# ignaschuemer7/soft-actor-critic

Hardware: AMD Instinct MI355X
Metric: SAC gradient steps/sec + replay-sample GB/s, BipedalWalker batch=256 (higher is better)
Workload: dtype fp32; 1 GPU; c2: BipedalWalker-v3 obs=24 act=4 2x[256, 256] MLPs, buffer=1000000, batch=256, auto-alpha, device sampler, fp32 arithmetic; global_batch=256, parallelism=replicas1, graph_chunk=64

## Files before the change

### soft-actor-critic_amd/csrc/sac_engine.hip

```cpp
#include "../../include/sac_engine.h"
#include "../../include/sac_engine_testing.h"

#include <algorithm>
#include <math.h>
#include <stdio.h>
#include <stdlib.h>
#include <string.h>
#include <string>
#include <vector>

#define SAC_VERSION "sac-mi355x 0.1.0"

#include "sac_phases.h"
#include "sac_split.h"
#include "sac_wide.h"
#include "sac_pairs.h"
#include "sac_envs.h"
#include "sac_plan.h"

template <typename T>
__global__ void pack_weights(const float* __restrict__ W, int K, int N, int Kp, int Np, T* __restrict__ Wc,
                             T* __restrict__ WTc) {
  for (int i = blockIdx.x * blockDim.x + threadIdx.x; i < Np * Kp; i += gridDim.x * blockDim.x) {
    const int n = i / Kp, k = i % Kp;
// ... 184 lines not shown

__host__ __device__ inline void eps_pair(uint64_t seed, uint64_t step, int b, int which, int p, int B, int A,
                                         float* out) {
  float n0, n1;
  philox_normal2(seed, step, (uint32_t)b, (uint32_t)which, (uint32_t)p, n0, n1);
  float* o = out + ((size_t)which * B + b) * A;
  o[2 * p] = n0;
  if (2 * p + 1 < A) o[2 * p + 1] = n1;
}
__global__ void eps_draw_kernel(uint64_t seed, uint64_t step, int B, int A, float* __restrict__ out) {
  const int NP = (A + 1) / 2;
  const int64_t n = 2LL * B * NP;
  for (int64_t i = blockIdx.x * (int64_t)blockDim.x + threadIdx.x; i < n; i += (int64_t)gridDim.x * blockDim.x) {
    const int p = (int)(i % NP);
    const int64_t rw = i / NP;
    eps_pair(seed, step, (int)(rw % B), (int)(rw / B), p, B, A, out);
  }
}

__global__ void replay_sample_kernel(const int64_t* __restrict__ state, int B, FeistelKeys fk, int32_t* __restrict__ out) {
  const int64_t size = state[0];
  const Feistel f = feistel_from_keys(fk, size);
  for (int b = blockIdx.x * blockDim.x + threadIdx.x; b < B; b += gridDim.x * blockDim.x)
    out[b] = (int32_t)feistel_sample(f, b, size);
}

static thread_local std::string g_err;
static int fail(int code, const std::string& msg) {
  g_err = msg;
  return code;
}
#define HIPCHK(x)                                                                                  \
  do {                                                                                             \
    hipError_t _e = (x);                                                                           \
    if (_e != hipSuccess) return fail(SAC_E_HIP, std::string(#x ": ") + hipGetErrorString(_e));    \
  } while (0)

static int validate(const sac_engine_config* c) {
  if (!c) return fail(SAC_E_INVALID, "null config");
  if (c->obs_dim < 1 || c->act_dim < 1 || c->act_dim > 32) return fail(SAC_E_INVALID, "obs_dim >= 1, 1 <= act_dim <= 32");
  if (c->batch < 1 || c->batch > (1 << 20)) return fail(SAC_E_INVALID, "batch out of range");
  if (c->q_layers < 2 || c->q_layers > SAC_DEV_LAYERS || c->pi_layers < 2 || c->pi_layers > SAC_DEV_LAYERS)
    return fail(SAC_E_INVALID, "networks need 1..5 hidden layers");
  if (c->q_dims[0] != c->obs_dim + c->act_dim || c->q_dims[c->q_layers] != 1)
    return fail(SAC_E_INVALID, "q_dims must run obs+act -> ... -> 1");
  if (c->pi_dims[0] != c->obs_dim || c->pi_dims[c->pi_layers] != 2 * c->act_dim)
    return fail(SAC_E_INVALID, "pi_dims must run obs -> ... -> 2*act");
  for (int i = 0; i <= c->q_layers; ++i)
    if (c->q_dims[i] < 1) return fail(SAC_E_INVALID, "bad q dim");
  for (int i = 0; i <= c->pi_layers; ++i)
    if (c->pi_dims[i] < 1) return fail(SAC_E_INVALID, "bad pi dim");
  const int acts[4] = {c->q_hidden_act, c->q_out_act, c->pi_hidden_act, c->pi_out_act};
  for (int a : acts)
    if (a < 0 || a > 6) return fail(SAC_E_INVALID, "bad activation code");
  if (c->precision != SAC_PREC_FP32 && c->precision != SAC_PREC_BF16) return fail(SAC_E_INVALID, "bad precision");
  if (c->layout < SAC_LAYOUT_AUTO || c->layout > SAC_LAYOUT_PAIRS || c->stage_path < -1 || c->stage_path > 1 ||
      c->stage_batch < -1 || c->stage_batch > 0 || c->upd_parts < 0 || c->upd_parts > 4 ||
      (c->upd_threads != 0 && c->upd_threads != 512 && c->upd_threads != 1024))
    return fail(SAC_E_INVALID, "bad layout override (layout 0..3, stage_path -1..1, stage_batch -1..0, "
                               "upd_parts 0..4, upd_threads 0 / 512 / 1024)");
  return SAC_OK;
}

template <typename T>
static void set_lds_attrs(size_t bytes) {
  (void)bytes;
  const int b = 160 * 1024;
  (void)hipFuncSetAttribute((const void*)sac_target_critic<T, false>, hipFuncAttributeMaxDynamicSharedMemorySize, b);
  (void)hipFuncSetAttribute((const void*)sac_target_critic<T, true>, hipFuncAttributeMaxDynamicSharedMemorySize, b);
  (void)hipFuncSetAttribute((const void*)sac_actor<T, false>, hipFuncAttributeMaxDynamicSharedMemorySize, b);
  (void)hipFuncSetAttribute((const void*)sac_actor<T, true>, hipFuncAttributeMaxDynamicSharedMemorySize, b);
  (void)hipFuncSetAttribute((const void*)sac_policy_act_kernel<T>, hipFuncAttributeMaxDynamicSharedMemorySize, b);
  (void)hipFuncSetAttribute((const void*)sac_rollout_step_kernel<T, false>, hipFuncAttributeMaxDynamicSharedMemorySize, b);
  (void)hipFuncSetAttribute((const void*)sac_rollout_step_kernel<T, true>, hipFuncAttributeMaxDynamicSharedMemorySize, b);
  (void)hipFuncSetAttribute((const void*)sac_rollout_step_dev_kernel<T, false>, hipFuncAttributeMaxDynamicSharedMemorySize,
                            b);
  (void)hipFuncSetAttribute((const void*)sac_rollout_step_dev_kernel<T, true>, hipFuncAttributeMaxDynamicSharedMemorySize,
                            b);
  (void)hipFuncSetAttribute((const void*)sac_q_values_kernel<T>, hipFuncAttributeMaxDynamicSharedMemorySize, b);
  (void)hipFuncSetAttribute((const void*)sac_target_critic_split<T>, hipFuncAttributeMaxDynamicSharedMemorySize, b);
  (void)hipFuncSetAttribute((const void*)sac_target_critic_pairs<T>, hipFuncAttributeMaxDynamicSharedMemorySize, b);
  (void)hipFuncSetAttribute((const void*)sac_actor_pairs<T>, hipFuncAttributeMaxDynamicSharedMemorySize, b);
  (void)hipFuncSetAttribute((const void*)sac_actor_split<T>, hipFuncAttributeMaxDynamicSharedMemorySize, b);
  (void)hipFuncSetAttribute((const void*)sac_critic_update<T>, hipFuncAttributeMaxDynamicSharedMemorySize, b);
  (void)hipFuncSetAttribute((const void*)sac_critic_update<T, 512>, hipFuncAttributeMaxDynamicSharedMemorySize, b);
  (void)hipFuncSetAttribute((const void*)sac_actor_update<T>, hipFuncAttributeMaxDynamicSharedMemorySize, b);
  (void)hipFuncSetAttribute((const void*)sac_wide_stage<T, WA_PLAIN, false>, hipFuncAttributeMaxDynamicSharedMemorySize, b);
  (void)hipFuncSetAttribute((const void*)sac_wide_stage<T, WA_ACT, false>, hipFuncAttributeMaxDynamicSharedMemorySize, b);
  (void)hipFuncSetAttribute((const void*)sac_wide_stage<T, WA_OUTBWD, false>, hipFuncAttributeMaxDynamicSharedMemorySize, b);
  (void)hipFuncSetAttribute((const void*)sac_wide_stage<T, WA_PLAIN, true>, hipFuncAttributeMaxDynamicSharedMemorySize, b);
  (void)hipFuncSetAttribute((const void*)sac_wide_stage<T, WA_ACT, true>, hipFuncAttributeMaxDynamicSharedMemorySize, b);
  (void)hipFuncSetAttribute((const void*)sac_wide_stage<T, WA_OUTBWD, true>, hipFuncAttributeMaxDynamicSharedMemorySize, b);
  (void)hipFuncSetAttribute((const void*)sac_wide_gather<T>, hipFuncAttributeMaxDynamicSharedMemorySize, b);
  (void)hipFuncSetAttribute((const void*)sac_wide_head<T>, hipFuncAttributeMaxDynamicSharedMemorySize, b);
}

__global__ void sac_noop_kernel() {}
__global__ void sac_spin_kernel(long long ticks) {
  const long long t0 = __builtin_amdgcn_s_memrealtime();
  while (__builtin_amdgcn_s_memrealtime() - t0 < ticks) __builtin_amdgcn_s_sleep(8);
}

#define BY_PRECISION(e, fn, ...) \
  ((e)->cfg.precision == SAC_PREC_BF16 ? fn<bf16>(__VA_ARGS__) : fn<float>(__VA_ARGS__))

template <typename T>
static void launch_kind(sac_engine* e, int kind, const sac_replay* rb, const int32_t* idx, const float* eps,
                        hipStream_t s) {
  const PhaseLaunch& L = e->launch[kind];
  switch (kind) {
    case L_A:
      switch (e->path) {
        case PATH_SPLIT: sac_target_critic_split<T><<<L.grid, L.threads, L.lds, s>>>(e->d, *rb, idx, eps); break;
        case PATH_ROLES: sac_target_critic<T, true><<<L.grid, L.threads, L.lds, s>>>(e->d, *rb, idx, eps); break;
        case PATH_PAIRS: sac_target_critic_pairs<T><<<L.grid, L.threads, L.lds, s>>>(e->d, *rb, idx, eps); break;
        case PATH_ROWS: sac_target_critic<T, false><<<L.grid, L.threads, L.lds, s>>>(e->d, *rb, idx, eps); break;
        case PATH_WIDE: break;
      }
      break;
    case L_B:
      if (L.threads == 512)
        sac_critic_update<T, 512><<<L.grid, 512, L.lds, s>>>(e->d, e->tilesB);
      else
        sac_critic_update<T><<<L.grid, L.threads, L.lds, s>>>(e->d, e->tilesB);
      break;
    case L_C:
      switch (e->path) {
        case PATH_SPLIT: sac_actor_split<T><<<L.grid, L.threads, L.lds, s>>>(e->d, *rb); break;
        case PATH_ROLES: sac_actor<T, true><<<L.grid, L.threads, L.lds, s>>>(e->d, *rb); break;
        case PATH_PAIRS: sac_actor_pairs<T><<<L.grid, L.threads, L.lds, s>>>(e->d, *rb); break;
        case PATH_ROWS: sac_actor<T, false><<<L.grid, L.threads, L.lds, s>>>(e->d, *rb); break;
        case PATH_WIDE: break;
      }
      break;
    case L_D:
      sac_actor_update<T><<<L.grid, L.threads, L.lds, s>>>(e->d, e->tilesD, e->nD);
      break;
  }
}

template <typename T>
static void launch_wide_stage(sac_engine* e, const sac_engine::WStage& st, const sac_replay* rb, const int32_t* idx,
                              const float* eps, hipStream_t s, bool stage_next, const int32_t* next_idx) {
  const size_t glds = (size_t)((WGR * (e->cfg.obs_dim + e->cfg.act_dim) + 1) & ~1) * 4 + WGR * 8;
  switch (st.kind) {
    case 0:
      sac_wide_gather<T><<<st.grid, WG_T, glds, s>>>(e->d, e->wdd, *rb, idx);
      break;
    case 1: {
      const int ng = st.last && stage_next ? (e->cfg.batch + WGR - 1) / WGR : 0;
      const int flags = st.last | (&st == &e->wst[1] ? 2 : 0) | (ng ? 4 : 0) | (int)((&st - e->wst.data()) << 8);
      const bool relu = e->cfg.q_hidden_act == ACT_RELU && e->cfg.pi_hidden_act == ACT_RELU;
      const int am = e->hostW[st.j0].amode;
      auto k = relu ? (am == WA_PLAIN ? sac_wide_stage<T, WA_PLAIN, true>
                       : am == WA_ACT ? sac_wide_stage<T, WA_ACT, true> : sac_wide_stage<T, WA_OUTBWD, true>)
                    : (am == WA_PLAIN ? sac_wide_stage<T, WA_PLAIN, false>
                       : am == WA_ACT ? sac_wide_stage<T, WA_ACT, false> : sac_wide_stage<T, WA_OUTBWD, false>);
      k<<<st.grid + ng, WG_T, std::max(st.lds, ng ? glds : 0), s>>>(e->d, e->wdd, e->wjobs + st.j0, st.j1 - st.j0,
                                                                    flags, st.grid, *rb, next_idx);
      break;
    }
    case 2:
      sac_wide_head<T><<<st.grid, WG_T, 0, s>>>(e->d, e->wdd, eps);
      break;
    case 3:
      launch_kind<T>(e, L_B, rb, idx, eps, s);
      break;
    case 4:
      launch_kind<T>(e, L_D, rb, idx, eps, s);
// ... 877 lines not shown
```

### soft-actor-critic_amd/csrc/sac_phases.h

```cpp
#pragma once
#include <type_traits>
#include <utility>

#include "sac_device.h"

#define SAC_DEV_LAYERS 6

__device__ __forceinline__ __amdgpu_buffer_rsrc_t coh_rsrc(const void* base, uint32_t bytes) {
  return __builtin_amdgcn_make_buffer_rsrc((void*)base, (short)0, (int)bytes, 0x00020000);
}
template <bool COH>
__device__ __forceinline__ void coh_store16(const void* base, uint32_t byte_off, u32x4 v) {
  __builtin_amdgcn_raw_buffer_store_b128(__builtin_bit_cast(__attribute__((ext_vector_type(4))) unsigned, v),
                                         coh_rsrc(base, 0xFFFFFFF0u), (int)byte_off, 0, COH ? 16 : 0);
}
__device__ __forceinline__ float coh_load(const float* p) {
  return __hip_atomic_load((float*)p, __ATOMIC_RELAXED, __HIP_MEMORY_SCOPE_AGENT);
}
template <bool COH>
__device__ __forceinline__ float ldf(const float* p) {
  if constexpr (COH) return coh_load(p);
  return *GPC(float, p);
}
__device__ __forceinline__ void coh_storef(float* p, float v) {
// ... 531 lines not shown
    lf* Pl = out ? Pout : (keepP ? lds + o_P[l] : nullptr);
    const int ldpl = out ? ldo : (keepP ? ldp[l] : 0);
    lf* Yl = out ? Yout : Y;
    const int ldyl = out ? ldo : ld;
    if (HELD && l == 0)
      layer_fwd<T, ROWS, 1>(X, ld, Ly, net.P + Ly.b_off, act, Pl, ldpl, Yl, ldyl, nullptr, 0, h0);
    else if (HELD && l == 1)
      layer_fwd<T, ROWS, 8>(X, ld, Ly, net.P + Ly.b_off, act, Pl, ldpl, Yl, ldyl, nullptr, 0, h1);
    else
      layer_fwd<T, ROWS>(X, ld, Ly, net.P + Ly.b_off, act, Pl, ldpl, Yl, ldyl, nullptr, 0);
    __syncthreads();
    lf* t = X;
    X = Y;
    Y = t;
  }
}

template <typename T, int ROWS, bool HELD = false>
__device__ __forceinline__ lf* mlp_backward(const AS_C NetDev& net, const lf* Gout, int ldo, lf* Xb, lf* Yb, int ld,
                                            const AS_C int* o_P, const AS_C int* ldp, lf* lds, bool storeGT, int Bp, int col0,
                                            int nvalid, const Held<T, 1>* h0 = nullptr,
                                            const Held<T, 8>* h1 = nullptr) {
  const int Lh = net.L - 1;
  const AS_C LayerDev& Lo = net.l[Lh];
  if (storeGT) store_T<T, ROWS>(Gout, ldo, Lo.Np, Lo.N, Lo.GT, Bp, col0, nvalid, Lo.dbp);
  layer_bwd<T, ROWS, HELD ? 1 : 0>(Gout, ldo, Lo, lds + o_P[Lh - 1], ldp[Lh - 1], net.hid_act, Yb, ld,
                                   (const Held<T, 1>*)h0);
  __syncthreads();
  lf* G = Yb;
  lf* Gn = Xb;
  for (int l = Lh - 1; l >= 0; --l) {
    const AS_C LayerDev& Ly = net.l[l];
    if (storeGT) store_T<T, ROWS>(G, ld, Ly.Np, Ly.N, Ly.GT, Bp, col0, nvalid, Ly.dbp);
    if (l == 0) break;
    if (HELD && l == Lh - 1)
      layer_bwd<T, ROWS, 8>(G, ld, Ly, lds + o_P[l - 1], ldp[l - 1], net.hid_act, Gn, ld, h1);
    else
      layer_bwd<T, ROWS>(G, ld, Ly, lds + o_P[l - 1], ldp[l - 1], net.hid_act, Gn, ld);
    __syncthreads();
    lf* t = G;
    G = Gn;
    Gn = t;
  }
  __syncthreads();
  return G;
}

#define LOG2F 0.69314718055994530942f
#define HALF_LOG_2PI 0.91893853320467274178f

__device__ __forceinline__ float fmin_nan(float a, float b) { return (a != a) ? a : (a < b ? a : b); }

template <typename T, int ROWS>
__device__ __forceinline__ void critic_unit_backward(const AS_C EngineDev& E, const AS_C NetDev& net, const lf* Gout, int ldo,
                                                     lf* lds) {
  const int Lh = net.L - 1;
  layer_bwd<T, ROWS>(Gout, ldo, net.l[Lh], lds + E.o_P1[Lh - 1], E.ldp1[Lh - 1], net.hid_act, lds + E.o_P2[Lh - 1],
                     E.ldp2[Lh - 1]);
  __syncthreads();
  for (int l = Lh - 1; l >= 1; --l) {
    layer_bwd<T, ROWS>(lds + E.o_P2[l], E.ldp2[l], net.l[l], lds + E.o_P1[l - 1], E.ldp1[l - 1], net.hid_act,
                       lds + E.o_P2[l - 1], E.ldp2[l - 1]);
    __syncthreads();
  }
}

__device__ __forceinline__ float adam_elem(float& p, float& m, float& v, float g, float w1, float b2, float w2,
                                           float bc2s, float eps, float neg_step) {
  const float mm = m + w1 * (g - m);
  float vv = v * b2;
  vv = vv + (w2 * g) * g;
  const float denom = sqrtf(vv) / bc2s + eps;
  const float pn = p + (neg_step * mm) / denom;
  m = mm;
  v = vv;
  p = pn;
  return pn;
}

#define SAC_UPD_THREADS 1024
#define SAC_UPD_BCH (512 / (int)sizeof(T))
#define SAC_UPD_SLOT_BYTES (64 * 528)
#define SAC_UPD_LDS_FOR(slots) ((slots) * SAC_UPD_SLOT_BYTES + 2 * 32 * 33 * 4 + 32 * 17 * 4 + (slots) * 256 * 4)
template <typename T, int UT, int GS = 1, int MS = 2>
__device__ __forceinline__ void dw_adam_tile(const AS_C EngineDev& E, const TileDesc* tdp_, bool polyak, int par,
                                             int par_x, lf* lds) {
  constexpr int KC = MM<T>::KC, KL = MM<T>::KL;
  constexpr int EPR = 16 / sizeof(T);
  constexpr int EPT = 1024 / UT;
  static_assert(EPR == KL, "a piece is one lane's fragment slice");
  const AS_C TileDesc& td = *(const AS_C TileDesc*)tdp_;
  STAMP(polyak ? 48 : 52);
  const int tid = threadIdx.x;
  const int Bp = td.bp;
  const int lds_row = SAC_UPD_BCH + 16 / (int)sizeof(T);
  AS_L T* stage = (AS_L T*)lds;
  const int nslot = E.upd_slots;
  constexpr int MAXS = MS, PPO = 32 * (SAC_UPD_BCH / EPR) / UT;
  const int ns = nslot < MAXS ? nslot : MAXS;
  const int slot_el = 64 * lds_row;
  lf* accs = lds + (ns * slot_el * (int)sizeof(T) + 15) / 16 * 4;
  lf* tgts = accs + 32 * 33;
  lf* red = tgts + 32 * 33;
  const float neg_step = GPC(float, E.adam_sc)[par * 6 + td.opt * 2];
  const float bc2s = GPC(float, E.adam_sc)[par * 6 + td.opt * 2 + 1];
  static_assert(PPO >= 1 && (32 * (SAC_UPD_BCH / EPR)) % UT == 0, "whole pieces per thread");
  const int rstep = ns * SAC_UPD_BCH;
  u32x4 rg[MAXS][GS + 1][PPO];
  const AS_G float* const seedp = GPC(float, td.seed);
  const bool lseeds = seedp && sizeof(T) == 4 && Bp > rstep;
  AS_L float* seedL = (AS_L float*)(red + 32 * 17);
  f32x4 sreg[MAXS];
  constexpr int SQ = EPR / 4;
  f32x4 sdr[MAXS][PPO][SQ];
  const AS_G T* const gsrc = GPC(T, td.GT);
  const AS_G T* const xsrc = GPC(T, td.XT) + par_x * td.xt_par;
  const long goff = GS > 1 ? td.goff : 0;
  const int ldg = td.ld, ldx = td.ldx;
  auto issue_seeds = [&](int r0, auto slc) __attribute__((always_inline)) {
    constexpr int sl = decltype(slc)::value;
    const int b0 = r0 + sl * SAC_UPD_BCH;
    if (lseeds && sl < ns && b0 < Bp) {
      const int bch = Bp - b0 < SAC_UPD_BCH ? Bp - b0 : SAC_UPD_BCH;
      if (threadIdx.x * 4 < bch) sreg[sl] = *(const AS_G f32x4*)(seedp + b0 + threadIdx.x * 4);
    }
  };
  auto issue = [&](int r0, auto slc, bool seeds = true) {
    constexpr int sl = decltype(slc)::value;
    const int b0 = r0 + sl * SAC_UPD_BCH;
    if (sl < ns && b0 < Bp) {
      const int bch = Bp - b0 < SAC_UPD_BCH ? Bp - b0 : SAC_UPD_BCH;
      const int per_row = bch / EPR;
      if (seeds) issue_seeds(r0, slc);
#pragma unroll
      for (int op = 0; op <= GS; ++op)
#pragma unroll
        for (int pi = 0; pi < PPO; ++pi) {
          const int i = threadIdx.x + pi * UT;
          const int row = i / per_row, pc = i % per_row;
          const AS_G T* src = op < GS ? gsrc + op * goff + (size_t)row * ldg : xsrc + (size_t)row * ldx;
          if (i < 32 * per_row) rg[sl][op][pi] = *(const AS_G u32x4*)(src + b0 + pc * EPR);
          if (op == 0 && seedp && !lseeds && i < 32 * per_row)
#pragma unroll
            for (int q = 0; q < SQ; ++q) sdr[sl][pi][q] = *(const AS_G f32x4*)(seedp + b0 + pc * EPR + 4 * q);
        }
    }
  };
  static_for<MAXS>([&](auto sl) { issue_seeds(0, sl); });
  static_for<MAXS>([&](auto sl) { issue(0, sl, false); });
  auto seeds_to_lds = [&](int r0) __attribute__((always_inline)) {
    if (lseeds)
      static_for<MAXS>([&](auto slc) {
        constexpr int sl = decltype(slc)::value;
        const int b0 = r0 + sl * SAC_UPD_BCH;
        if (sl < ns && b0 < Bp) {
          const int bch = Bp - b0 < SAC_UPD_BCH ? Bp - b0 : SAC_UPD_BCH;
          if (tid * 4 < bch) *(AS_L f32x4*)(seedL + sl * SAC_UPD_BCH + tid * 4) = sreg[sl];
        }
      });
  };
  AS_G float* W = GP(float, td.W);
  AS_G float* Wm = GP(float, td.Wm);
  AS_G float* Wv = GP(float, td.Wv);
  AS_G float* tW = GP(float, td.tW);
  float p[EPT], m[EPT], v[EPT], tp[EPT];
  size_t idx[EPT];
  bool ok[EPT];
#pragma unroll
  for (int e = 0; e < EPT; ++e) {
    const int el = tid + e * UT, en = el >> 5, ek = el & 31;
    const int n = td.n0 + en, k = td.k0 + ek;
    ok[e] = n < td.N && k < td.K;
    idx[e] = ok[e] ? (size_t)n * td.K + k : 0;
    if (td.kpart < 2) {
      p[e] = W[idx[e]];
      m[e] = Wm[idx[e]];
      v[e] = Wv[idx[e]];
      tp[e] = polyak ? tW[idx[e]] : 0.f;
    } else {
      p[e] = m[e] = v[e] = tp[e] = 0.f;
    }
  }
  const bool do_bias = td.k0 == 0 && td.kpart <= 1;
  const bool bias_acc = td.k0 == 0;
  float pb = 0.f, mb = 0.f, vb = 0.f, tbv = 0.f;
  if (do_bias && tid < 32 && td.n0 + tid < td.N) {
    pb = GPC(float, td.b)[td.n0 + tid];
    mb = GPC(float, td.bm)[td.n0 + tid];
    vb = GPC(float, td.bv)[td.n0 + tid];
    if (polyak) tbv = GPC(float, td.tb)[td.n0 + tid];
  }
  constexpr int BPT = (512 + UT - 1) / UT;
  float bsum[BPT];
#pragma unroll
  for (int j = 0; j < BPT; ++j) bsum[j] = 0.f;
  const int lane = tid & 63, wave = wave_id();
  const int c = lane & 15, g = lane >> 4;
  constexpr int KQ = 4, NWV = UT / 64, PPW = 16 / NWV;
  static_assert(UT % 64 == 0 && 16 % NWV == 0, "16 (sub-tile, K-quarter) pairs over whole waves");
  f32x4 acc[PPW];
#pragma unroll
  for (int j = 0; j < PPW; ++j) acc[j] = f32x4{0.f, 0.f, 0.f, 0.f};
  seeds_to_lds(0);
  if (lseeds) __syncthreads();
  for (int r0 = 0; r0 < Bp; r0 += rstep) {
    static_for<MAXS>([&](auto slc) {
      constexpr int sl = decltype(slc)::value;
      const int b0 = r0 + sl * SAC_UPD_BCH;
      if (sl < ns && b0 < Bp) {
        const int bch = Bp - b0 < SAC_UPD_BCH ? Bp - b0 : SAC_UPD_BCH;
        const int per_row = bch / EPR;
#pragma unroll
        for (int op = 0; op < 2; ++op)
#pragma unroll
          for (int pi = 0; pi < PPO; ++pi) {
            const int i = tid + pi * UT;
            const int row = i / per_row + 32 * op, pc = i % per_row;
            u32x4 v = rg[sl][op ? GS : 0][pi];
            if constexpr (sizeof(T) == 4) {
              if constexpr (GS > 1)
                if (op == 0) {
                  f32x4 a = __builtin_bit_cast(f32x4, v);
#pragma unroll
                  for (int q = 1; q < GS; ++q) a += __builtin_bit_cast(f32x4, rg[sl][q][pi]);
                  v = __builtin_bit_cast(u32x4, a);
                }
              if (op == 0 && seedp)
                v = __builtin_bit_cast(u32x4, __builtin_bit_cast(f32x4, v) *
                                                  (lseeds ? *(const AS_L f32x4*)(seedL + sl * SAC_UPD_BCH + pc * EPR)
                                                          : sdr[sl][pi][0]));
            } else if (op == 0 && (GS > 1 || seedp)) {
              bf16x8 h = __builtin_bit_cast(bf16x8, v);
              float a[8];
#pragma unroll
              for (int e = 0; e < 8; ++e) a[e] = (float)h[e];
#pragma unroll
              for (int q = 1; q < GS; ++q) {
                const bf16x8 hq = __builtin_bit_cast(bf16x8, rg[sl][q][pi]);
#pragma unroll
                for (int e = 0; e < 8; ++e) a[e] += (float)hq[e];
              }
              if (seedp)
#pragma unroll
                for (int e = 0; e < 8; ++e) a[e] *= sdr[sl][pi][e >> 2][e & 3];
#pragma unroll
              for (int e = 0; e < 8; ++e) h[e] = (bf16)a[e];
              v = __builtin_bit_cast(u32x4, h);
            }
            if (i < 32 * per_row) *(AS_L u32x4*)(stage + sl * slot_el + row * lds_row + pc * EPR) = v;
          }
        issue(r0 + rstep, slc);
        __syncthreads();
        if (r0 == 0 && sl == 0) STAMP(polyak ? 51 : 55);
        if (bias_acc) {
#pragma unroll
          for (int j = 0; j < BPT; ++j) {
            const int t = tid + j * UT, bn = t >> 4, bs = t & 15;
            if (t < 512)
              for (int c = bs * EPR; c < bch; c += 16 * EPR) {
                const AS_L T* q = stage + sl * slot_el + bn * lds_row + c;
                if constexpr (sizeof(T) == 4) {
                  const f32x4 x = *(const AS_L f32x4*)q;
                  bsum[j] += (x[0] + x[1]) + (x[2] + x[3]);
                } else {
                  const bf16x8 x = *(const AS_L bf16x8*)q;
                  float s = 0.f;
#pragma unroll
                  for (int e = 0; e < 8; ++e) s += (float)x[e];
                  bsum[j] += s;
                }
              }
          }
        }
#pragma unroll
        for (int j = 0; j < PPW; ++j) {
          const int pr = wave + j * NWV, kq = pr >> 2;
          const int ns = ((pr & 3) >> 1) * 16, ks = (pr & 1) * 16;
          const AS_L T* arow = stage + sl * slot_el + (ns + c) * lds_row + g * KL;
          const AS_L T* brow = stage + sl * slot_el + (32 + ks + c) * lds_row + g * KL;
          for (int ch = kq; ch < bch / KC; ch += KQ) {
            typename MM<T>::Frag a, b;
            if constexpr (sizeof(T) == 2) {
              a = *(const AS_L bf16x8*)(arow + ch * KC);
              b = *(const AS_L bf16x8*)(brow + ch * KC);
            } else {
              a = *(const AS_L f32x4*)(arow + ch * KC);
              b = *(const AS_L f32x4*)(brow + ch * KC);
            }
            MM<T>::mma(acc[j], a, b);
          }
        }
      }
    });
    seeds_to_lds(r0 + rstep);
    __syncthreads();
  }
  STAMP(polyak ? 49 : 53);
  {
#pragma unroll
    for (int j = 0; j < PPW; ++j) {
      const int pr = wave + j * NWV;
      const int ns = ((pr & 3) >> 1) * 16, ks = (pr & 1) * 16;
      lf* part = (lf*)stage + (pr >> 2) * (32 * 33);
#pragma unroll
      for (int i = 0; i < 4; ++i) part[(ns + g * 4 + i) * 33 + ks + c] = acc[j][i];
    }
  }
  __syncthreads();
  for (int el = tid; el < 1024; el += UT) {
    const int o = (el >> 5) * 33 + (el & 31);
    const lf* part = (const lf*)stage;
    float sum = part[o];
#pragma unroll
    for (int q = 1; q < KQ; ++q) sum += part[q * (32 * 33) + o];
    accs[o] = sum;
  }
#pragma unroll
  for (int j = 0; j < BPT; ++j) {
    const int t = tid + j * UT;
    if (bias_acc && t < 512) red[(t >> 4) * 17 + (t & 15)] = bsum[j];
  }
  __syncthreads();
  constexpr int MAXP = UT == 512 ? 7 : 3;
  float gbx[MAXP];
#pragma unroll
  for (int q = 0; q < MAXP; ++q) gbx[q] = 0.f;
  if (td.kpart) {
    const uint32_t ep = *GPC(uint32_t, E.sync) + 1u;
    if (td.kpart >= 2) {
      AS_G uint64_t* mine = GP(uint64_t, td.part) + (size_t)(td.kpart - 2) * SAC_PART_STRIDE;
      for (int el = tid; el < 1024; el += UT) {
        const uint64_t x = (uint64_t)__float_as_uint(accs[(el >> 5) * 33 + (el & 31)]) | ((uint64_t)ep << 32);
        __hip_atomic_store((uint64_t*)(mine + el), x, __ATOMIC_RELAXED, __HIP_MEMORY_SCOPE_AGENT);
      }
      if (bias_acc && tid < 32) {
        float gb = 0.f;
        for (int q = 0; q < 16; ++q) gb += red[tid * 17 + q];
        const uint64_t x = (uint64_t)__float_as_uint(gb) | ((uint64_t)ep << 32);
        __hip_atomic_store((uint64_t*)(mine + 1024 + tid), x, __ATOMIC_RELAXED, __HIP_MEMORY_SCOPE_AGENT);
      }
      return;
    }
    constexpr int EL = 1024 / UT;
    static_assert(EL * UT == 1024 && EL <= 4, "granules per thread");
    const int np = td.nparts - 1;
    const bool pb_here = do_bias && tid < 32;
    float v[MAXP][EL];
    for (int it = 0;; ++it) {
      bool all = true;
#pragma unroll
      for (int q = 0; q < MAXP; ++q)
        if (q < np) {
#pragma unroll
          for (int j = 0; j < EL; ++j) {
            const uint64_t x = __hip_atomic_load(td.part + (size_t)q * SAC_PART_STRIDE + tid + j * UT,
                                                 __ATOMIC_RELAXED, __HIP_MEMORY_SCOPE_AGENT);
            all = all && (uint32_t)(x >> 32) == ep;
            v[q][j] = __uint_as_float((uint32_t)x);
          }
          if (pb_here) {
            const uint64_t x = __hip_atomic_load(td.part + (size_t)q * SAC_PART_STRIDE + 1024 + tid,
                                                 __ATOMIC_RELAXED, __HIP_MEMORY_SCOPE_AGENT);
            all = all && (uint32_t)(x >> 32) == ep;
            gbx[q] = __uint_as_float((uint32_t)x);
          }
        }
      if (all) break;
      if (it > E.spin_limit) {
        __hip_atomic_store((uint32_t*)GP(uint32_t, E.sync) + 1 , 1u, __ATOMIC_RELAXED,
                           __HIP_MEMORY_SCOPE_AGENT);
        break;
      }
      __builtin_amdgcn_s_sleep(1);
    }
#pragma unroll
    for (int j = 0; j < EL; ++j) {
      const int el = tid + j * UT, o = (el >> 5) * 33 + (el & 31);
      float sum = accs[o];
#pragma unroll
      for (int q = 0; q < MAXP; ++q)
        if (q < np) sum += v[q][j];
      accs[o] = sum;
    }
    __syncthreads();
  }
  STAMP(polyak ? 50 : 54);
  const float w1 = (float)(1.0 - (double)E.beta1), b2 = E.beta2, w2 = (float)(1.0 - (double)E.beta2);
  const float eps = E.adam_eps, tau = E.tau, omt = (float)(1.0 - (double)E.tau);
  float pn[EPT], tn[EPT];
#pragma unroll
  for (int e = 0; e < EPT; ++e) {
    const int el = tid + e * UT;
    pn[e] = 0.f;
    tn[e] = 0.f;
    if (ok[e]) {
      pn[e] = adam_elem(p[e], m[e], v[e], accs[(el >> 5) * 33 + (el & 31)], w1, b2, w2, bc2s, eps, neg_step);
      W[idx[e]] = p[e];
      Wm[idx[e]] = m[e];
      Wv[idx[e]] = v[e];
      if (polyak) {
        tn[e] = tau * pn[e] + omt * tp[e];
        tW[idx[e]] = tn[e];
      }
    }
  }
  __syncthreads();
#pragma unroll
  for (int e = 0; e < EPT; ++e) {
    const int el = tid + e * UT;
    accs[(el >> 5) * 33 + (el & 31)] = pn[e];
    if (polyak) tgts[(el >> 5) * 33 + (el & 31)] = tn[e];
  }
  if (do_bias && tid < 32 && td.n0 + tid < td.N) {
    float gb = 0.f;
    for (int q = 0; q < 16; ++q) gb += red[tid * 17 + q];
    if (td.kpart) {
#pragma unroll
      for (int q = 0; q < MAXP; ++q)
        if (q < td.nparts - 1) gb += gbx[q];
    }
    const float pbn = adam_elem(pb, mb, vb, gb, w1, b2, w2, bc2s, eps, neg_step);
    GP(float, td.b)[td.n0 + tid] = pb;
    GP(float, td.bm)[td.n0 + tid] = mb;
    GP(float, td.bv)[td.n0 + tid] = vb;
    if (polyak) GP(float, td.tb)[td.n0 + tid] = tau * pbn + omt * tbv;
  }
  __syncthreads();
  constexpr int PPR = 32 / EPR;
  for (int mat = 0; mat < (polyak ? 3 : 2); ++mat) {
    const void* base = mat == 0 ? td.Wc : mat == 1 ? td.WTc : td.tWc;
    for (int i = tid; i < 32 * PPR; i += UT) {
      const int row = i / PPR, pc = i % PPR;
      T vv[EPR];
      size_t off;
      if (mat == 1) {
#pragma unroll
        for (int j = 0; j < EPR; ++j) vv[j] = MM<T>::cvt(accs[(pc * EPR + j) * 33 + row]);
        off = packed_off<T>(td.k0 + row, td.n0 + pc * EPR, td.Np);
      } else {
        const lf* srcm = mat == 0 ? accs : tgts;
#pragma unroll
        for (int j = 0; j < EPR; ++j) vv[j] = MM<T>::cvt(srcm[row * 33 + pc * EPR + j]);
        off = packed_off<T>(td.n0 + row, td.k0 + pc * EPR, td.Kp);
      }
      coh_store16<false>(base, (uint32_t)(off * sizeof(T)), *(const u32x4*)vv);
    }
  }
}

template <typename T, int UT, int MS = 2>
__device__ __forceinline__ void dw_adam_tile_any(const AS_C EngineDev& E, const TileDesc* tdp_, bool polyak, int par,
                                                 int par_x, lf* lds) {
  if constexpr (UT != 512) {
    const int gs = ((const AS_C TileDesc*)tdp_)->gsum;
    if constexpr (sizeof(T) == 4)
      if (gs == 4) return dw_adam_tile<T, UT, 4, MS>(E, tdp_, polyak, par, par_x, lds);
    if (gs == 2) return dw_adam_tile<T, UT, 2, MS>(E, tdp_, polyak, par, par_x, lds);
  }
  dw_adam_tile<T, UT, 1, MS>(E, tdp_, polyak, par, par_x, lds);
}

__device__ __forceinline__ void alpha_and_losses(const AS_C EngineDev& E, int par, lf* red) {
  const int tid = threadIdx.x, NT = blockDim.x, B = E.B;
  const float H = E.target_entropy;
  AS_G double* st = GP(double, E.alpha_state);
  const double st0 = st[0];
  const float la32 = (float)st0;
  const float mB = -1.0f / (float)B;
  const AS_G float* lp = GPC(float, E.lp_st) + par * E.Br;
  const AS_G float* lossp = GPC(float, E.lossp) + par * E.nrt * 4;
  float sg = 0.f, sl = 0.f, l0 = 0.f, l1 = 0.f, l2 = 0.f;
  for (int b = tid; b < B; b += NT) {
    const float term = lp[b] + H;
    sg += mB * term;
    sl += la32 * term;
  }
  for (int rt = tid; rt < E.nrt; rt += NT) {
    l0 += lossp[rt * 4 + 0];
    l1 += lossp[rt * 4 + 1];
    l2 += lossp[rt * 4 + 2];
  }
  red[0 * NT + tid] = sg;
  red[1 * NT + tid] = sl;
  red[2 * NT + tid] = l0;
  red[3 * NT + tid] = l1;
  red[4 * NT + tid] = l2;
  __syncthreads();
  for (int s = NT / 2; s > 0; s >>= 1) {
    if (tid < s)
// ... 988 lines not shown
```

Before: 20720 gradient steps/s.

## Add single-pass dW+Adam path with batched LDS fragment loads and static partials

Result: faster. 21120 gradient steps/s (median of 6 runs) (+1.9%).

```diff
diff --git a/soft-actor-critic_amd/csrc/sac_engine.hip b/soft-actor-critic_amd/csrc/sac_engine.hip
--- a/soft-actor-critic_amd/csrc/sac_engine.hip
+++ b/soft-actor-critic_amd/csrc/sac_engine.hip
@@ -290,9 +290,10 @@
   (void)hipFuncSetAttribute((const void*)sac_target_critic_pairs<T>, hipFuncAttributeMaxDynamicSharedMemorySize, b);
   (void)hipFuncSetAttribute((const void*)sac_actor_pairs<T>, hipFuncAttributeMaxDynamicSharedMemorySize, b);
   (void)hipFuncSetAttribute((const void*)sac_actor_split<T>, hipFuncAttributeMaxDynamicSharedMemorySize, b);
-  (void)hipFuncSetAttribute((const void*)sac_critic_update<T>, hipFuncAttributeMaxDynamicSharedMemorySize, b);
+  const int bu = b - SAC_UPD_PART_BYTES;
+  (void)hipFuncSetAttribute((const void*)sac_critic_update<T>, hipFuncAttributeMaxDynamicSharedMemorySize, bu);
   (void)hipFuncSetAttribute((const void*)sac_critic_update<T, 512>, hipFuncAttributeMaxDynamicSharedMemorySize, b);
-  (void)hipFuncSetAttribute((const void*)sac_actor_update<T>, hipFuncAttributeMaxDynamicSharedMemorySize, b);
+  (void)hipFuncSetAttribute((const void*)sac_actor_update<T>, hipFuncAttributeMaxDynamicSharedMemorySize, bu);
   (void)hipFuncSetAttribute((const void*)sac_wide_stage<T, WA_PLAIN, false>, hipFuncAttributeMaxDynamicSharedMemorySize, b);
   (void)hipFuncSetAttribute((const void*)sac_wide_stage<T, WA_ACT, false>, hipFuncAttributeMaxDynamicSharedMemorySize, b);
   (void)hipFuncSetAttribute((const void*)sac_wide_stage<T, WA_OUTBWD, false>, hipFuncAttributeMaxDynamicSharedMemorySize, b);
diff --git a/soft-actor-critic_amd/csrc/sac_phases.h b/soft-actor-critic_amd/csrc/sac_phases.h
--- a/soft-actor-critic_amd/csrc/sac_phases.h
+++ b/soft-actor-critic_amd/csrc/sac_phases.h
@@ -637,6 +637,11 @@
 #define SAC_UPD_BCH (512 / (int)sizeof(T))
 #define SAC_UPD_SLOT_BYTES (64 * 528)
 #define SAC_UPD_LDS_FOR(slots) ((slots) * SAC_UPD_SLOT_BYTES + 2 * 32 * 33 * 4 + 32 * 17 * 4 + (slots) * 256 * 4)
+#define SAC_UPD_PART_BYTES (4 * 32 * 33 * 4)
+__device__ __forceinline__ lf* upd_partials() {
+  __shared__ float part[SAC_UPD_PART_BYTES / 4];
+  return (lf*)part;
+}
 template <typename T, int UT, int GS = 1, int MS = 2>
 __device__ __forceinline__ void dw_adam_tile(const AS_C EngineDev& E, const TileDesc* tdp_, bool polyak, int par,
                                              int par_x, lf* lds) {
@@ -758,124 +763,225 @@
   for (int j = 0; j < PPW; ++j) acc[j] = f32x4{0.f, 0.f, 0.f, 0.f};
   seeds_to_lds(0);
   if (lseeds) __syncthreads();
-  for (int r0 = 0; r0 < Bp; r0 += rstep) {
-    static_for<MAXS>([&](auto slc) {
-      constexpr int sl = decltype(slc)::value;
-      const int b0 = r0 + sl * SAC_UPD_BCH;
-      if (sl < ns && b0 < Bp) {
-        const int bch = Bp - b0 < SAC_UPD_BCH ? Bp - b0 : SAC_UPD_BCH;
-        const int per_row = bch / EPR;
-#pragma unroll
-        for (int op = 0; op < 2; ++op)
-#pragma unroll
-          for (int pi = 0; pi < PPO; ++pi) {
-            const int i = tid + pi * UT;
-            const int row = i / per_row + 32 * op, pc = i % per_row;
-            u32x4 v = rg[sl][op ? GS : 0][pi];
-            if constexpr (sizeof(T) == 4) {
-              if constexpr (GS > 1)
-                if (op == 0) {
-                  f32x4 a = __builtin_bit_cast(f32x4, v);
-#pragma unroll
-                  for (int q = 1; q < GS; ++q) a += __builtin_bit_cast(f32x4, rg[sl][q][pi]);
-                  v = __builtin_bit_cast(u32x4, a);
-                }
-              if (op == 0 && seedp)
-                v = __builtin_bit_cast(u32x4, __builtin_bit_cast(f32x4, v) *
-                                                  (lseeds ? *(const AS_L f32x4*)(seedL + sl * SAC_UPD_BCH + pc * EPR)
-                                                          : sdr[sl][pi][0]));
-            } else if (op == 0 && (GS > 1 || seedp)) {
-              bf16x8 h = __builtin_bit_cast(bf16x8, v);
-              float a[8];
-#pragma unroll
-              for (int e = 0; e < 8; ++e) a[e] = (float)h[e];
-#pragma unroll
-              for (int q = 1; q < GS; ++q) {
-                const bf16x8 hq = __builtin_bit_cast(bf16x8, rg[sl][q][pi]);
-#pragma unroll
-                for (int e = 0; e < 8; ++e) a[e] += (float)hq[e];
-              }
-              if (seedp)
-#pragma unroll
-                for (int e = 0; e < 8; ++e) a[e] *= sdr[sl][pi][e >> 2][e & 3];
-#pragma unroll
-              for (int e = 0; e < 8; ++e) h[e] = (bf16)a[e];
-              v = __builtin_bit_cast(u32x4, h);
+  auto stage_slot = [&](auto slc, int bch) __attribute__((always_inline)) {
+    constexpr int sl = decltype(slc)::value;
+    const int per_row = bch / EPR;
+#pragma unroll
+    for (int op = 0; op < 2; ++op)
+#pragma unroll
+      for (int pi = 0; pi < PPO; ++pi) {
+        const int i = tid + pi * UT;
+        const int row = i / per_row + 32 * op, pc = i % per_row;
+        u32x4 v = rg[sl][op ? GS : 0][pi];
+        if constexpr (sizeof(T) == 4) {
+          if constexpr (GS > 1)
+            if (op == 0) {
+              f32x4 a = __builtin_bit_cast(f32x4, v);
+#pragma unroll
+              for (int q = 1; q < GS; ++q) a += __builtin_bit_cast(f32x4, rg[sl][q][pi]);
+              v = __builtin_bit_cast(u32x4, a);
             }
-            if (i < 32 * per_row) *(AS_L u32x4*)(stage + sl * slot_el + row * lds_row + pc * EPR) = v;
+          if (op == 0 && seedp)
+            v = __builtin_bit_cast(u32x4, __builtin_bit_cast(f32x4, v) *
+                                              (lseeds ? *(const AS_L f32x4*)(seedL + sl * SAC_UPD_BCH + pc * EPR)
+                                                      : sdr[sl][pi][0]));
+        } else if (op == 0 && (GS > 1 || seedp)) {
+          bf16x8 h = __builtin_bit_cast(bf16x8, v);
+          float a[8];
+#pragma unroll
+          for (int e = 0; e < 8; ++e) a[e] = (float)h[e];
+#pragma unroll
+          for (int q = 1; q < GS; ++q) {
+            const bf16x8 hq = __builtin_bit_cast(bf16x8, rg[sl][q][pi]);
+#pragma unroll
+            for (int e = 0; e < 8; ++e) a[e] += (float)hq[e];
           }
-        issue(r0 + rstep, slc);
-        __syncthreads();
-        if (r0 == 0 && sl == 0) STAMP(polyak ? 51 : 55);
-        if (bias_acc) {
-#pragma unroll
-          for (int j = 0; j < BPT; ++j) {
-            const int t = tid + j * UT, bn = t >> 4, bs = t & 15;
-            if (t < 512)
-              for (int c = bs * EPR; c < bch; c += 16 * EPR) {
-                const AS_L T* q = stage + sl * slot_el + bn * lds_row + c;
+          if (seedp)
+#pragma unroll
+            for (int e = 0; e < 8; ++e) a[e] *= sdr[sl][pi][e >> 2][e & 3];
+#pragma unroll
+          for (int e = 0; e < 8; ++e) h[e] = (bf16)a[e];
+          v = __builtin_bit_cast(u32x4, h);
+        }
+        if (i < 32 * per_row) *(AS_L u32x4*)(stage + sl * slot_el + row * lds_row + pc * EPR) = v;
+      }
+  };
+  constexpr int NIT = SAC_UPD_BCH / KC / KQ;
+  constexpr int NBP = SAC_UPD_BCH / (16 * EPR);
+  bool single = false;
+  if constexpr (UT == SAC_UPD_THREADS) single = Bp <= rstep;
+  float gel[EPT];
+  if (single) {
+    if constexpr (UT == SAC_UPD_THREADS) {
+      static_assert(PPW == 1 && BPT == 1, "one (sub-tile, K-quarter) pair per wave");
+      typedef typename MM<T>::Frag Frag;
+      static_for<MAXS>([&](auto slc) {
+        constexpr int sl = decltype(slc)::value;
+        const int b0 = sl * SAC_UPD_BCH;
+        if (sl < ns && b0 < Bp) stage_slot(slc, Bp - b0 < SAC_UPD_BCH ? Bp - b0 : SAC_UPD_BCH);
+      });
+      __syncthreads();
+      STAMP(polyak ? 51 : 55);
+      const int kq = wave >> 2, sn = ((wave & 3) >> 1) * 16, sk = (wave & 1) * 16;
+      const int bn = tid >> 4, bs = tid & 15;
+      const bool bias_lane = bias_acc && tid < 512;
+      auto dw_and_bias = [&](auto fullc) __attribute__((always_inline)) {
+        constexpr bool FULL = decltype(fullc)::value;
+        Frag fa[MAXS][NIT], fb[MAXS][NIT], bx[MAXS][NBP];
+        auto slots = [&](auto&& f) __attribute__((always_inline)) {
+          static_for<MAXS>([&](auto slc) {
+            constexpr int sl = decltype(slc)::value;
+            const int b0 = sl * SAC_UPD_BCH;
+            if (sl < ns && b0 < Bp)
+              f(slc, FULL || Bp - b0 >= SAC_UPD_BCH ? SAC_UPD_BCH : Bp - b0);
+          });
+        };
+        slots([&](auto slc, int bch) {
+          constexpr int sl = decltype(slc)::value;
+          const AS_L T* arow = stage + sl * slot_el + (sn + c) * lds_row + g * KL;
+          const AS_L T* brow = stage + sl * slot_el + (32 + sk + c) * lds_row + g * KL;
+#pragma unroll
+          for (int it = 0; it < NIT; ++it) {
+            const int ch = kq + it * KQ;
+            if (FULL || ch < bch / KC) {
+              fa[sl][it] = *(const AS_L Frag*)(arow + ch * KC);
+              fb[sl][it] = *(const AS_L Frag*)(brow + ch * KC);
+            }
+          }
+        });
+        if (bias_lane)
+          slots([&](auto slc, int bch) {
+            constexpr int sl = decltype(slc)::value;
+#pragma unroll
+            for (int it = 0; it < NBP; ++it) {
+              const int bc = (bs + it * 16) * EPR;
+              if (FULL || bc < bch) bx[sl][it] = *(const AS_L Frag*)(stage + sl * slot_el + bn * lds_row + bc);
+            }
+          });
+        slots([&](auto slc, int bch) {
+          constexpr int sl = decltype(slc)::value;
+#pragma unroll
+          for (int it = 0; it < NIT; ++it)
+            if (FULL || kq + it * KQ < bch / KC) MM<T>::mma(acc[0], fa[sl][it], fb[sl][it]);
+        });
+        if (bias_lane)
+          slots([&](auto slc, int bch) {
+            constexpr int sl = decltype(slc)::value;
+#pragma unroll
+            for (int it = 0; it < NBP; ++it)
+              if (FULL || (bs + it * 16) * EPR < bch) {
+                const Frag x = bx[sl][it];
                 if constexpr (sizeof(T) == 4) {
-                  const f32x4 x = *(const AS_L f32x4*)q;
-                  bsum[j] += (x[0] + x[1]) + (x[2] + x[3]);
+                  bsum[0] += (x[0] + x[1]) + (x[2] + x[3]);
                 } else {
-                  const bf16x8 x = *(const AS_L bf16x8*)q;
                   float s = 0.f;
 #pragma unroll
                   for (int e = 0; e < 8; ++e) s += (float)x[e];
-                  bsum[j] += s;
+                  bsum[0] += s;
                 }
               }
+          });
+      };
+      if (Bp % SAC_UPD_BCH == 0)
+        dw_and_bias(std::true_type{});
+      else
+        dw_and_bias(std::false_type{});
+      STAMP(polyak ? 49 : 53);
+      lf* part = upd_partials();
+#pragma unroll
+      for (int i = 0; i < 4; ++i) part[kq * (32 * 33) + (sn + g * 4 + i) * 33 + sk + c] = acc[0][i];
+      if (bias_lane) red[bn * 17 + bs] = bsum[0];
+      __syncthreads();
+#pragma unroll
+      for (int e = 0; e < EPT; ++e) {
+        const int el = tid + e * UT, o = (el >> 5) * 33 + (el & 31);
+        float sum = part[o];
+#pragma unroll
+        for (int q = 1; q < KQ; ++q) sum += part[q * (32 * 33) + o];
+        gel[e] = sum;
+      }
+    }
+  } else {
+    for (int r0 = 0; r0 < Bp; r0 += rstep) {
+      static_for<MAXS>([&](auto slc) {
+        constexpr int sl = decltype(slc)::value;
+        const int b0 = r0 + sl * SAC_UPD_BCH;
+        if (sl < ns && b0 < Bp) {
+          const int bch = Bp - b0 < SAC_UPD_BCH ? Bp - b0 : SAC_UPD_BCH;
+          stage_slot(slc, bch);
+          issue(r0 + rstep, slc);
+          __syncthreads();
+          if (r0 == 0 && sl == 0) STAMP(polyak ? 51 : 55);
+          if (bias_acc) {
+#pragma unroll
+            for (int j = 0; j < BPT; ++j) {
+              const int t = tid + j * UT, bn = t >> 4, bs = t & 15;
+              if (t < 512)
+                for (int c = bs * EPR; c < bch; c += 16 * EPR) {
+                  const AS_L T* q = stage + sl * slot_el + bn * lds_row + c;
+                  if constexpr (sizeof(T) == 4) {
+                    const f32x4 x = *(const AS_L f32x4*)q;
+                    bsum[j] += (x[0] + x[1]) + (x[2] + x[3]);
+                  } else {
+                    const bf16x8 x = *(const AS_L bf16x8*)q;
+                    float s = 0.f;
+#pragma unroll
+                    for (int e = 0; e < 8; ++e) s += (float)x[e];
+                    bsum[j] += s;
+                  }
+                }
+            }
+          }
+#pragma unroll
+          for (int j = 0; j < PPW; ++j) {
+            const int pr = wave + j * NWV, kq = pr >> 2;
+            const int ns = ((pr & 3) >> 1) * 16, ks = (pr & 1) * 16;
+            const AS_L T* arow = stage + sl * slot_el + (ns + c) * lds_row + g * KL;
+            const AS_L T* brow = stage + sl * slot_el + (32 + ks + c) * lds_row + g * KL;
+            for (int ch = kq; ch < bch / KC; ch += KQ) {
+              typename MM<T>::Frag a, b;
+              if constexpr (sizeof(T) == 2) {
+                a = *(const AS_L bf16x8*)(arow + ch * KC);
+                b = *(const AS_L bf16x8*)(brow + ch * KC);
+              } else {
+                a = *(const AS_L f32x4*)(arow + ch * KC);
+                b = *(const AS_L f32x4*)(brow + ch * KC);
+              }
+              MM<T>::mma(acc[j], a, b);
+            }
           }
         }
-#pragma unroll
-        for (int j = 0; j < PPW; ++j) {
-          const int pr = wave + j * NWV, kq = pr >> 2;
-          const int ns = ((pr & 3) >> 1) * 16, ks = (pr & 1) * 16;
-          const AS_L T* arow = stage + sl * slot_el + (ns + c) * lds_row + g * KL;
-          const AS_L T* brow = stage + sl * slot_el + (32 + ks + c) * lds_row + g * KL;
-          for (int ch = kq; ch < bch / KC; ch += KQ) {
-            typename MM<T>::Frag a, b;
-            if constexpr (sizeof(T) == 2) {
-              a = *(const AS_L bf16x8*)(arow + ch * KC);
-              b = *(const AS_L bf16x8*)(brow + ch * KC);
-            } else {
-              a = *(const AS_L f32x4*)(arow + ch * KC);
-              b = *(const AS_L f32x4*)(brow + ch * KC);
-            }
-            MM<T>::mma(acc[j], a, b);
-          }
-        }
-      }
-    });
-    seeds_to_lds(r0 + rstep);
+      });
+      seeds_to_lds(r0 + rstep);
+      __syncthreads();
+    }
+    STAMP(polyak ? 49 : 53);
+    {
+#pragma unroll
+      for (int j = 0; j < PPW; ++j) {
+        const int pr = wave + j * NWV;
+        const int ns = ((pr & 3) >> 1) * 16, ks = (pr & 1) * 16;
+        lf* part = (lf*)stage + (pr >> 2) * (32 * 33);
+#pragma unroll
+        for (int i = 0; i < 4; ++i) part[(ns + g * 4 + i) * 33 + ks + c] = acc[j][i];
+      }
+    }
     __syncthreads();
-  }
-  STAMP(polyak ? 49 : 53);
-  {
-#pragma unroll
-    for (int j = 0; j < PPW; ++j) {
-      const int pr = wave + j * NWV;
-      const int ns = ((pr & 3) >> 1) * 16, ks = (pr & 1) * 16;
-      lf* part = (lf*)stage + (pr >> 2) * (32 * 33);
-#pragma unroll
-      for (int i = 0; i < 4; ++i) part[(ns + g * 4 + i) * 33 + ks + c] = acc[j][i];
-    }
-  }
-  __syncthreads();
-  for (int el = tid; el < 1024; el += UT) {
-    const int o = (el >> 5) * 33 + (el & 31);
-    const lf* part = (const lf*)stage;
-    float sum = part[o];
-#pragma unroll
-    for (int q = 1; q < KQ; ++q) sum += part[q * (32 * 33) + o];
-    accs[o] = sum;
-  }
-#pragma unroll
-  for (int j = 0; j < BPT; ++j) {
-    const int t = tid + j * UT;
-    if (bias_acc && t < 512) red[(t >> 4) * 17 + (t & 15)] = bsum[j];
-  }
-  __syncthreads();
+    for (int el = tid; el < 1024; el += UT) {
+      const int o = (el >> 5) * 33 + (el & 31);
+      const lf* part = (const lf*)stage;
+      float sum = part[o];
+#pragma unroll
+      for (int q = 1; q < KQ; ++q) sum += part[q * (32 * 33) + o];
+      accs[o] = sum;
+    }
+#pragma unroll
+    for (int j = 0; j < BPT; ++j) {
+      const int t = tid + j * UT;
+      if (bias_acc && t < 512) red[(t >> 4) * 17 + (t & 15)] = bsum[j];
+    }
+    __syncthreads();
+  }
   constexpr int MAXP = UT == 512 ? 7 : 3;
   float gbx[MAXP];
 #pragma unroll
@@ -884,8 +990,11 @@
     const uint32_t ep = *GPC(uint32_t, E.sync) + 1u;
     if (td.kpart >= 2) {
       AS_G uint64_t* mine = GP(uint64_t, td.part) + (size_t)(td.kpart - 2) * SAC_PART_STRIDE;
-      for (int el = tid; el < 1024; el += UT) {
-        const uint64_t x = (uint64_t)__float_as_uint(accs[(el >> 5) * 33 + (el & 31)]) | ((uint64_t)ep << 32);
+#pragma unroll
+      for (int e = 0; e < EPT; ++e) {
+        const int el = tid + e * UT;
+        const float dw = single ? gel[e] : accs[(el >> 5) * 33 + (el & 31)];
+        const uint64_t x = (uint64_t)__float_as_uint(dw) | ((uint64_t)ep << 32);
         __hip_atomic_store((uint64_t*)(mine + el), x, __ATOMIC_RELAXED, __HIP_MEMORY_SCOPE_AGENT);
       }
       if (bias_acc && tid < 32) {
@@ -931,13 +1040,16 @@
 #pragma unroll
     for (int j = 0; j < EL; ++j) {
       const int el = tid + j * UT, o = (el >> 5) * 33 + (el & 31);
-      float sum = accs[o];
+      float sum = single ? gel[j] : accs[o];
 #pragma unroll
       for (int q = 0; q < MAXP; ++q)
         if (q < np) sum += v[q][j];
-      accs[o] = sum;
-    }
-    __syncthreads();
+      if (single)
+        gel[j] = sum;
+      else
+        accs[o] = sum;
+    }
+    if (!single) __syncthreads();
   }
   STAMP(polyak ? 50 : 54);
   const float w1 = (float)(1.0 - (double)E.beta1), b2 = E.beta2, w2 = (float)(1.0 - (double)E.beta2);
@@ -949,7 +1061,8 @@
     pn[e] = 0.f;
     tn[e] = 0.f;
     if (ok[e]) {
-      pn[e] = adam_elem(p[e], m[e], v[e], accs[(el >> 5) * 33 + (el & 31)], w1, b2, w2, bc2s, eps, neg_step);
+      const float dw = single ? gel[e] : accs[(el >> 5) * 33 + (el & 31)];
+      pn[e] = adam_elem(p[e], m[e], v[e], dw, w1, b2, w2, bc2s, eps, neg_step);
       W[idx[e]] = p[e];
       Wm[idx[e]] = m[e];
       Wv[idx[e]] = v[e];
@@ -959,7 +1072,7 @@
       }
     }
   }
-  __syncthreads();
+  if (!single) __syncthreads();
 #pragma unroll
   for (int e = 0; e < EPT; ++e) {
     const int el = tid + e * UT;
```
